# isarandi/metro-pose3d

Hardware: AMD Instinct MI355X
Metric: crops/sec (256x256, RN50 stride16) (higher is better)
Workload: dtype f16

## Files before the change

metro_pose3d_amd/csrc/conv_b1.hip:

```cpp
#include "metro_common.h"
#include "gfx950_prims.h"

namespace metro {

namespace b1 {
constexpr int NPROD = 8, NCONS = 4, NT = 64 * (NPROD + NCONS), TN = 64, K = 64, CB = 256, C2 = 64, NBUF = 3;
constexpr int X_BYTES = TN * 128;
constexpr int OUT_ROW = CB * 2 + 16;
constexpr int OUT_BYTES = TN * OUT_ROW;
constexpr int W1S_ROW = CB * 2 + 16;
static_assert(48 * W1S_ROW <= OUT_BYTES, "W1's stage must fit the second output tile");
template <bool REB>
struct Lay {
    static constexpr int NIN = REB ? 3 : 2;
    static constexpr int X_OFF = 0;
    static constexpr int OUT_OFF = NBUF * NIN * X_BYTES;
    static constexpr int PAR_OFF = OUT_OFF + 2 * OUT_BYTES;
    static constexpr int B3 = 0, BSC = 1024, BB = 2048, B2 = 3072, PRO = 3328, SC2 = 3584, SH2 = 4096, PAR_BYTES = 4608;
    static constexpr int W1T_OFF = PAR_OFF + PAR_BYTES;
    static constexpr int LDS = W1T_OFF + 8 * 64 * 16;
};
}

struct B1Args {
// ... 4 lines not shown
    const half_t* w_sc;
    const float* bias_sc;
    const half_t* pro_scale;
    const half_t* pro_shift;
    const half_t* in_b;
    const half_t* w_b;
    const float* bias_b;
    const half_t* w2;
    const float* bias2;
    const half_t* scale2;
    const half_t* shift2;
    half_t* out;
    half_t* out_sub;
    half_t* out2;
    int m_total, n_tiles;
    int h_out, w_out, lw_out, sub_off, h_sub, w_sub;
};

template <bool REB, int OUTM>
__global__ __launch_bounds__(b1::NT) void conv_b1_chain_kernel(B1Args a) {
    using namespace b1;
    using L = Lay<REB>;
    constexpr int NIN = L::NIN;
    extern __shared__ __attribute__((aligned(16))) char smem[];
    const unsigned smem_base = lds_offset_of(smem);
    const int tid = threadIdx.x;
    const int lane = tid & 63;
    const int wave = __builtin_amdgcn_readfirstlane(tid >> 6);
    const bool producer = wave < NPROD;
    const int G = gridDim.x;
    const int t0 = blockIdx.x;
    if (t0 >= a.n_tiles) return;
    const int T = (a.n_tiles - t0 + G - 1) / G;
    char* par = smem + L::PAR_OFF;
    {
        float* f = reinterpret_cast<float*>(par);
        if (tid < 256) {
            f[L::B3 / 4 + tid] = a.bias[tid];
            f[L::BSC / 4 + tid] = a.bias_sc[tid];
            if (REB) f[L::BB / 4 + tid] = a.bias_b[tid];
            reinterpret_cast<half_t*>(par + L::SC2)[tid] = a.scale2[tid];
            reinterpret_cast<half_t*>(par + L::SH2)[tid] = a.shift2[tid];
        }
        if (tid < 512) {
            const int ks = tid >> 6, ln = tid & 63;
            *reinterpret_cast<uint4*>(smem + L::W1T_OFF + tid * 16) =
                *reinterpret_cast<const uint4*>(a.w2 + (size_t)(48 + (ln & 15)) * CB + ks * 32 + (ln >> 4) * 8);
        }
        for (int c = tid; c < 48 * 32; c += NT)
            *reinterpret_cast<uint4*>(smem + L::OUT_OFF + OUT_BYTES + (c >> 5) * W1S_ROW + (c & 31) * 16) =
                *reinterpret_cast<const uint4*>(a.w2 + (size_t)(c >> 5) * CB + (c & 31) * 8);
        if (tid < 64) {
            f[L::B2 / 4 + tid] = a.bias2[tid];
            reinterpret_cast<half_t*>(par + L::PRO)[tid] = a.pro_scale[tid];
            reinterpret_cast<half_t*>(par + L::PRO)[64 + tid] = a.pro_shift[tid];
        }
    }
    const int frag_row = lane & 31, frag_half = lane >> 5;

    if (producer) {
        half8_t wf[4], wsf[4], wbf[4];
        static_assert(NPROD * W_STAGE_BYTES <= L::OUT_OFF + OUT_BYTES, "the staging scratch must stay below the second output tile (W1's stage)");
        load_w_frags_staged<K>(a.w + (size_t)wave * 32 * K, wf, smem + wave * W_STAGE_BYTES, lane);
        load_w_frags_staged<K>(a.w_sc + (size_t)wave * 32 * K, wsf, smem + wave * W_STAGE_BYTES, lane);
        if constexpr (REB) load_w_frags_staged<K>(a.w_b + (size_t)wave * 32 * K, wbf, smem + wave * W_STAGE_BYTES, lane);
#pragma unroll
        for (int kk = 0; kk < 4; ++kk) {
            asm volatile("" : "+v"(wf[kk]), "+v"(wsf[kk]));
            if constexpr (REB) asm volatile("" : "+v"(wbf[kk]));
        }
        const int xrow = wave * 8 + (lane >> 3);
        const int xoff = xrow * K + (((lane & 7) ^ swz<64>(xrow)) * 8);
        auto issue_tile = [&](int tile, int slot) {
            const size_t m0 = (size_t)tile * TN;
            const unsigned dst = smem_base + L::X_OFF + slot * NIN * X_BYTES + wave * 1024;
            dma16(a.in + m0 * K + xoff, __builtin_amdgcn_readfirstlane(dst));
            dma16(a.x_sc + m0 * K + xoff, __builtin_amdgcn_readfirstlane(dst + X_BYTES));
            if constexpr (REB) dma16(a.in_b + m0 * K + xoff, __builtin_amdgcn_readfirstlane(dst + 2 * X_BYTES));
        };
        wait_vm_and_barrier<0>();
        half8_t pre_s, pre_b;
        {
            const int ch = ((lane & 7) ^ swz<64>(xrow)) * 8;
            pre_s = *reinterpret_cast<const half8_t*>(par + L::PRO + ch * 2);
            pre_b = *reinterpret_cast<const half8_t*>(par + L::PRO + 128 + ch * 2);
        }
        issue_tile(t0, 0);
        if (T > 1) issue_tile(t0 + G, 1);
        floatx4 b3_r[4];
#pragma unroll
        for (int q = 0; q < 4; ++q) b3_r[q] = *reinterpret_cast<const floatx4*>(par + L::B3 + (wave * 32 + 8 * q + 4 * frag_half) * 4);
        const float* bias_sc_l = reinterpret_cast<const float*>(par + L::BSC);
        const float* bias_b_l = reinterpret_cast<const float*>(par + L::BB);
        const int boff0 = frag_row * 128 + ((frag_half ^ swz<64>(frag_row)) << 4);
        int slot = 0;
        for (int j = 0; j <= T; ++j) {
            if (j < T) {
                if (j + 1 < T) wait_vm<NIN>();
                else wait_vm<0>();
            }
            if (j < T) {
                half8_t* mine = reinterpret_cast<half8_t*>(smem + L::X_OFF + (slot * NIN + 1) * X_BYTES + wave * 1024 + lane * 16);
                const half8_t z = {};
                *mine = __builtin_elementwise_max(*mine * pre_s + pre_b, z);
            }
            wait_lgkm_and_barrier();
            if (j + 2 < T) issue_tile(t0 + (j + 2) * G, slot >= 1 ? slot - 1 : 2);
            if (j < T) {
                const char* xs = smem + L::X_OFF + slot * NIN * X_BYTES;
                char* ot = smem + L::OUT_OFF + (j & 1) * OUT_BYTES;
                floatx16 acc[2];
                half4_t xsum[2][4];
#pragma unroll
                for (int p = 0; p < 2; ++p)
#pragma unroll
                    for (int e = 0; e < 16; ++e) acc[p][e] = 0.f;
#pragma unroll
                for (int kk = 0; kk < 4; ++kk)
#pragma unroll
                    for (int p = 0; p < 2; ++p) {
                        const half8_t bs = *reinterpret_cast<const half8_t*>(xs + X_BYTES + p * 4096 + (boff0 ^ (kk << 5)));
// ... 158 lines not shown
```

metro_pose3d_amd/csrc/conv_pw64.hip:

```cpp
#include <cstdlib>
#include <type_traits>

#include "metro_common.h"
#include "gfx950_prims.h"

namespace metro {

struct Pw64Args {
    const half_t* in;
    const half_t* w;
    const float* bias;
    const half_t* pro_scale;
    const half_t* pro_shift;
    const half_t* residual;
    half_t* out;
    const half_t* w2;
    const float* bias2;
    const half_t* scale2;
    const half_t* shift2;
    half_t* out2;
    const half_t* x_sc;
    const half_t* w_sc;
    const float* bias_sc;
    const half_t* in_b;
// ... 7 lines not shown
};

namespace pw {
constexpr int NW = 8, NT = 512;
template <int K, int WM, int CB = 256>
struct Lay {
    static constexpr int WN = NW / WM;
    static constexpr int NI = CB / 32 / WM;
    static constexpr int TN = 32 * WN;
    static constexpr int KS = K / 64;
    static constexpr int SL_BYTES = TN * 128;
    static constexpr int X_BYTES = KS * SL_BYTES;
    static constexpr int XI = X_BYTES / 1024 / NW;
    static constexpr int CPR = CB / 8;
    static constexpr int RI = TN * CPR / NT;
    static constexpr int OUT_ROW = CB * 2 + 16;
    static constexpr int OUT_BYTES = TN * OUT_ROW;
    static constexpr int RES_BYTES = TN * CB * 2;
    static constexpr int C2 = CB == 512 ? 128 : 64;
    static constexpr int BIAS2_OFF = CB * 4, PRO_OFF = BIAS2_OFF + 512, BSC_OFF = PRO_OFF + 4 * K, BB_OFF = BSC_OFF + 1024;
    static constexpr int PAR_BYTES = BB_OFF + 1024;
    static constexpr int X_OFF = 0;
    static constexpr int OUT_OFF = X_OFF + 2 * X_BYTES;
    static constexpr int PAR_OFF = OUT_OFF + OUT_BYTES;
    static constexpr int RES_OFF = PAR_OFF + PAR_BYTES;
    static_assert(X_BYTES % (1024 * NW) == 0, "input tile must split evenly over the waves");
    static_assert(NI >= 1 && RI >= 1 && (TN * CPR) % NT == 0, "tile / thread mismatch");
};
template <int K, int WM, bool RES, int MODE2, bool PSC = false, int CB = 256, bool REB = false>
constexpr int lds_bytes() {
    return Lay<K, WM, CB>::RES_OFF + (RES ? 2 * Lay<K, WM, CB>::RES_BYTES : PSC ? (REB ? 4 : 2) * Lay<K, WM, CB>::X_BYTES
                                      : (MODE2 == 1 && K > 64) ? Lay<K, WM, CB>::C2 * (2 * K + 16) + Lay<K, WM, CB>::TN * (2 * Lay<K, WM, CB>::C2 + 16) : 0);
}
}

template <int BASE, int MAXX>
__device__ __forceinline__ void pw_wait_vm_plus(int extra) {
    if constexpr (MAXX == 0) {
        wait_vm<BASE>();
    } else {
        if (extra >= MAXX) wait_vm<BASE + MAXX>();
        else pw_wait_vm_plus<BASE, MAXX - 1>(extra);
    }
}
__device__ __forceinline__ void pw_wait_lgkm2(half8_t& r, half8_t& r2, int n) {
    switch (n) {
        case 0: asm volatile("s_waitcnt lgkmcnt(0)" : "+v"(r), "+v"(r2)); break;
        case 2: asm volatile("s_waitcnt lgkmcnt(2)" : "+v"(r), "+v"(r2)); break;
        case 4: asm volatile("s_waitcnt lgkmcnt(4)" : "+v"(r), "+v"(r2)); break;
        default: asm volatile("s_waitcnt lgkmcnt(6)" : "+v"(r), "+v"(r2)); break;
    }
}

template <int K, int WM, bool PRO, bool RES, int MODE2, bool RSUB = false, bool PSC = false, int CB = 256, bool REB = false, int OUTM = 0>
__global__ __launch_bounds__(pw::NT) void conv_pw64_kernel(Pw64Args a) {
    using namespace pw;
    using L = Lay<K, WM, CB>;
    static_assert((WM == 4 && K <= 128) || (WM == 8 && K <= 512), "weights must fit the register file as MFMA fragments");
    static_assert(CB == 256 || (CB == 512 && K == 128 && WM == 8 && RES && !PRO && !RSUB) ||
                      (CB == 512 && K == 256 && WM == 8 && !RES && PRO && MODE2 == 1),
                  "512-channel blocks: conv3 of block2, or block2's projection shortcut + conv1 pair");
    static_assert(MODE2 == 0 || (K == 64 && WM == 4) || (MODE2 == 2 && CB == 512) || (MODE2 == 1 && CB == 512 && K == 256),
                  "second outputs: block1 shapes, conv3 + next conv1 of block2, or block2's pair");
    static_assert(!PSC || (MODE2 == 2 && !PRO && !RES), "in-launch projection shortcut: conv3 + next conv1 of block1/unit_1");
    static_assert(!REB || PSC, "rebuilt residual: on top of the in-launch projection shortcut");
    static_assert(OUTM == 0 || (MODE2 == 2 && PSC), "outputs kept on chip: the conv3 + next conv1 launches of block1");
    constexpr int KK = K / 16, WN = L::WN, NI = L::NI, TN = L::TN, XI = L::XI, RI = L::RI;
    constexpr int X_BYTES = L::X_BYTES, X_OFF = L::X_OFF, OUT_OFF = L::OUT_OFF, PAR_OFF = L::PAR_OFF, RES_OFF = L::RES_OFF,
                  RES_BYTES = L::RES_BYTES, SL_BYTES = L::SL_BYTES, OUT_ROW = L::OUT_ROW, CPR = L::CPR, C2 = L::C2;
    extern __shared__ __attribute__((aligned(16))) char smem[];
    const unsigned smem_base = lds_offset_of(smem);
    constexpr int XS_OFF = RES_OFF;
    constexpr int XB_OFF = XS_OFF + 2 * X_BYTES;

    const int tid = threadIdx.x;
    const int lane = tid & 63;
    const int wave = __builtin_amdgcn_readfirstlane(tid >> 6);
    const int wm = wave / WN, wn = wave % WN;
    const int frag_row = lane & 31, frag_half = lane >> 5;
    const int halves = a.c_out / CB;
    const int G = gridDim.x / halves;
    int half, t;
    if ((gridDim.x & 7) == 0 && ((gridDim.x >> 3) % halves) == 0) {
        const int xcd = blockIdx.x & 7, j = blockIdx.x >> 3;
        half = j % halves;
        t = xcd * ((gridDim.x >> 3) / halves) + j / halves;
    } else {
        half = blockIdx.x % halves;
        t = blockIdx.x / halves;
    }
    if (t >= a.n_tiles) return;
    a.w += (size_t)half * CB * K;
    a.bias += half * CB;
    a.out += half * CB;
    if (RES) a.residual += half * CB;
    const int ldo = a.c_out;
    const half_t* zero = reinterpret_cast<const half_t*>(g_zero_page);

    half8_t wf[NI][KK];
    constexpr bool W_STAGED = K >= 128 && pw::lds_bytes<K, WM, RES, MODE2, PSC, CB, REB>() >= NW * W_STAGE_BYTES;
    constexpr int RG = C2 / 16;
    constexpr int NTW = TN / 16 / (NW / RG);
    constexpr int KS2 = CB / 32;
    half8_t w2r[MODE2 == 2 ? KS2 : 1];
    if constexpr (W_STAGED) {
#pragma unroll
        for (int i = 0; i < NI; ++i)
            load_w_frags_staged<K>(a.w + (size_t)((wm * NI + i) * 32) * K, wf[i], smem + wave * W_STAGE_BYTES, lane);
        if constexpr (MODE2 == 2) load_w_frags16_staged<CB>(a.w2 + (size_t)((wave % RG) * 16) * CB, w2r, smem + wave * W_STAGE_BYTES, lane);
        __syncthreads();
    } else {
#pragma unroll
        for (int i = 0; i < NI; ++i)
#pragma unroll
            for (int kk = 0; kk < KK; ++kk)
                wf[i][kk] = *reinterpret_cast<const half8_t*>(a.w + (size_t)((wm * NI + i) * 32 + frag_row) * K + kk * 16 + frag_half * 8);
    }
    half8_t wsf[NI][KK];
    if constexpr (PSC) {
#pragma unroll
        for (int i = 0; i < NI; ++i)
#pragma unroll
            for (int kk = 0; kk < KK; ++kk)
                wsf[i][kk] = *reinterpret_cast<const half8_t*>(a.w_sc + (size_t)((wm * NI + i) * 32 + frag_row) * K + kk * 16 + frag_half * 8);
    }
    half8_t wbf[NI][KK];
    if constexpr (REB) {
#pragma unroll
        for (int i = 0; i < NI; ++i)
#pragma unroll
            for (int kk = 0; kk < KK; ++kk)
                wbf[i][kk] = *reinterpret_cast<const half8_t*>(a.w_b + (size_t)((wm * NI + i) * 32 + frag_row) * K + kk * 16 + frag_half * 8);
    }
    constexpr bool W2_LDS = MODE2 == 1 && K > 64;
    constexpr bool PREPASS = PRO && W2_LDS;
    constexpr int W2_ROW = 2 * K + 16;
    constexpr int W2_OFF = RES_OFF;
    constexpr int O2_ROW = 2 * C2 + 16, O2_OFF = W2_OFF + C2 * W2_ROW;
    half8_t w2f[MODE2 == 1 && !W2_LDS ? KK : 1];
    if constexpr (MODE2 == 1 && !W2_LDS) {
        if (wave < 4) {
#pragma unroll
            for (int kk = 0; kk < KK; ++kk)
                w2f[kk] = *reinterpret_cast<const half8_t*>(a.w2 + (size_t)(wm * 32 + frag_row) * K + kk * 16 + frag_half * 8);
        }
    }
    if constexpr (W2_LDS) {
        for (int c = tid; c < C2 * (K / 8); c += NT) {
            const int r = c / (K / 8), q = c % (K / 8);
            *reinterpret_cast<uint4*>(smem + W2_OFF + r * W2_ROW + q * 16) = *reinterpret_cast<const uint4*>(a.w2 + (size_t)r * K + q * 8);
        }
    }
    const char* w2l = smem + W2_OFF + (wm * 32 + frag_row) * W2_ROW + frag_half * 16;
    float* bias_l = reinterpret_cast<float*>(smem + PAR_OFF);
    float* bias2_l = reinterpret_cast<float*>(smem + PAR_OFF + L::BIAS2_OFF);
    half_t* pro_l = reinterpret_cast<half_t*>(smem + PAR_OFF + L::PRO_OFF);
    if (tid < CB) bias_l[tid] = a.bias[tid];
    if (MODE2 != 0 && tid < C2) bias2_l[tid] = a.bias2[tid];
    if ((PRO || PSC) && tid < K) { pro_l[tid] = a.pro_scale[tid]; pro_l[K + tid] = a.pro_shift[tid]; }
    float* bias_sc_l = reinterpret_cast<float*>(smem + PAR_OFF + L::BSC_OFF);
    if (PSC && tid < 256) bias_sc_l[tid] = a.bias_sc[tid];
    float* bias_b_l = reinterpret_cast<float*>(smem + PAR_OFF + L::BB_OFF);
    if (REB && tid < 256) bias_b_l[tid] = a.bias_b[tid];
    const int ch = tid & (CPR - 1);
    half8_t sc2 = {}, sh2 = {};
    if constexpr (MODE2 == 2) {
        sc2 = *reinterpret_cast<const half8_t*>(a.scale2 + ch * 8);
        sh2 = *reinterpret_cast<const half8_t*>(a.shift2 + ch * 8);
        if constexpr (!W_STAGED) {
#pragma unroll
            for (int ks = 0; ks < KS2; ++ks)
                w2r[ks] = *reinterpret_cast<const half8_t*>(a.w2 + (size_t)((wave % RG) * 16 + (lane & 15)) * CB + ks * 32 + (lane >> 4) * 8);
        }
    }

    int xrow[XI], xoff[XI];
#pragma unroll
    for (int i = 0; i < XI; ++i) {
        const int q = i * NW + wave;
        xrow[i] = (q % (TN / 8)) * 8 + (lane >> 3);
        xoff[i] = xrow[i] * K + (q / (TN / 8)) * 64 + (((lane & 7) ^ swz<64>(xrow[i])) * 8);
    }
    auto issue_tile = [&](int tile, int buf) {
        const int m0 = tile * TN;
#pragma unroll
        for (int i = 0; i < XI; ++i) {
            const half_t* xs = (m0 + xrow[i] < a.m_total) ? a.in + (size_t)m0 * K + xoff[i] : zero;
            dma16(xs, __builtin_amdgcn_readfirstlane(smem_base + X_OFF + buf * X_BYTES + (i * NW + wave) * 1024));
            if constexpr (PSC) {
                const half_t* ss = (m0 + xrow[i] < a.m_total) ? a.x_sc + (size_t)m0 * K + xoff[i] : zero;
                dma16(ss, __builtin_amdgcn_readfirstlane(smem_base + XS_OFF + buf * X_BYTES + (i * NW + wave) * 1024));
            }
            if constexpr (REB) {
                const half_t* sb = (m0 + xrow[i] < a.m_total) ? a.in_b + (size_t)m0 * K + xoff[i] : zero;
                dma16(sb, __builtin_amdgcn_readfirstlane(smem_base + XB_OFF + buf * X_BYTES + (i * NW + wave) * 1024));
            }
        }
        if constexpr (RES) {
#pragma unroll
            for (int it = 0; it < RI; ++it) {
                const int c = it * NT + tid;
                const int m = m0 + c / CPR;
                size_t rrow = m;
                if constexpr (RSUB) {
                    const int hw = a.h_out * a.w_out;
                    const int img = m / hw, rem = m - img * hw;
                    const int ho = rem / a.w_out, wo = rem - ho * a.w_out;
                    rrow = ((size_t)img * a.res_h + a.res_off + a.res_stride * ho) * a.res_w + a.res_off + a.res_stride * wo;
                }
                const half_t* rs = m < a.m_total ? a.residual + rrow * ldo + (c & (CPR - 1)) * 8 : zero;
                dma16(rs, __builtin_amdgcn_readfirstlane(smem_base + RES_OFF + buf * RES_BYTES + it * 8192 + wave * 1024));
            }
        }
    };

    issue_tile(t, 0);
    constexpr int S2 = MODE2 == 2 ? NTW : (MODE2 == 1 && K > 64) ? 1 : 4;
    constexpr int RS = OUTM == 0 ? RI : 0;
    const bool two = MODE2 == 2 || (MODE2 == 1 && (wave < 4 || K > 64));
    bool prev_full = false;
    int prev_sub = 0;
    for (int it = 0;; ++it, t += G) {
        const int buf = it & 1;
        const int m0 = t * TN;
        if (it == 0 || !prev_full) wait_vm<0>();
        else if constexpr (OUTM == 2) pw_wait_vm_plus<S2, RI>(prev_sub);
        else if (two) wait_vm<RS + S2>();
        else wait_vm<RS>();
        wait_lgkm_and_barrier();
        if (t + G < a.n_tiles) issue_tile(t + G, buf ^ 1);
        prev_full = m0 + TN <= a.m_total;

        if constexpr (PREPASS) {
            static_assert(X_BYTES / 16 == 2 * NT, "two 16-byte chunks of the input tile per thread");
            const int c8 = lane & 7, prow = (wave & 3) * 8 + (lane >> 3);
            const half8_t z = {};
#pragma unroll
            for (int h = 0; h < 2; ++h) {
                const int sl = (wave >> 2) + 2 * h;
                half8_t* xp = reinterpret_cast<half8_t*>(smem + X_OFF + buf * X_BYTES + sl * SL_BYTES + prow * 128 + ((c8 ^ swz<64>(prow)) << 4));
                const half8_t sc = *reinterpret_cast<const half8_t*>(pro_l + sl * 64 + c8 * 8);
                const half8_t sh = *reinterpret_cast<const half8_t*>(pro_l + K + sl * 64 + c8 * 8);
                *xp = __builtin_elementwise_max(*xp * sc + sh, z);
            }
            wait_lgkm_and_barrier();
        }
        floatx16 acc[NI], acc2, accs[NI];
#pragma unroll
        for (int e = 0; e < 16; ++e) {
// ... 266 lines not shown
                         d.res_offset + 2 * (d.w_out - 1) < d.res_w;
    if (d.has_residual && !res_plain && !(f.form == ConvForm::Plain && res_sub && d.c_in <= 128)) return false;
    switch (f.form) {
        case ConvForm::Pair: {
            static const int pair256 = tuning_knob("METRO_PW_PAIR256", 1);
            return ((d.c_in == 64 && d.c_out == 320) || (pair256 && !classic_forms_forced() && d.c_in == 256 && d.c_out == 640)) &&
                   d.has_prologue && !d.has_residual && f.pair.relu2 == 1 && 5 * f.pair.c_out2 == d.c_out && f.pair.split == 4 * f.pair.c_out2;
        }
        case ConvForm::Next: {
            static const int next128 = tuning_knob("METRO_PW_NEXT128", 1);
            return ((d.c_in == 64 && d.c_out == 256 && f.next.c2 == 64) ||
                    (next128 && d.c_in == 128 && d.c_out == 512 && res_plain && f.next.c2 == 128)) && !d.has_prologue && d.has_residual;
        }
        case ConvForm::NextProj:
        case ConvForm::NextRebuild:
            return d.c_in == 64 && d.c_out == 256 && !d.has_prologue && !d.has_residual && f.next.c2 == 64 &&
                   (f.form == ConvForm::NextProj || b1_map_ok(d));
        case ConvForm::Plain:
            break;
    }
    if (d.c_in == 64 && d.c_out == 256) return (d.has_prologue != 0) != (d.has_residual != 0);
    static const int maxk = tuning_knob("METRO_PW_MAXK", 512);
    return (d.c_in == 128 || d.c_in == 256 || d.c_in == 512) && d.c_in <= maxk && d.c_out == 4 * d.c_in &&
           !d.has_prologue && d.has_residual;
}

template <int K, int WM, bool PRO, bool RES, int MODE2, bool RSUB = false, bool PSC = false, int CB = 256, bool REB = false, int OUTM = 0>
static int launch_pw(Pw64Args a, hipStream_t stream) {
    if (note_kernel("conv_pw64<k%d,wm%d%s%s%s%s%s%s%s%s>", K, WM, CB == 512 ? ",cb512" : "", PRO ? ",pro" : "", RES ? ",res" : "",
                    MODE2 == 1 ? ",pair" : MODE2 == 2 ? ",next" : "", RSUB ? ",ressub" : "", PSC ? ",projsc" : "", REB ? ",rebuild" : "",
                    OUTM == 1 ? ",noout" : OUTM == 2 ? ",subout" : ""))
        return METRO_OK;
    auto kern = conv_pw64_kernel<K, WM, PRO, RES, MODE2, RSUB, PSC, CB, REB, OUTM>;
    constexpr int lds = pw::lds_bytes<K, WM, RES, MODE2, PSC, CB, REB>();
    a.n_tiles = (a.m_total + pw::Lay<K, WM, CB>::TN - 1) / pw::Lay<K, WM, CB>::TN;
    static PerDeviceInt cap;
    int grid_cap = 0;
    if (const int st = ensure_dyn_lds_and_grid_cap(reinterpret_cast<const void*>(kern), pw::NT, lds, cap, "conv_pw64",
                                                   tuning_knob("METRO_PW64_BPC", 0) , &grid_cap))
        return st;
    const int halves = a.c_out / CB;
    int grid = a.n_tiles * halves < grid_cap ? a.n_tiles * halves : grid_cap;
    grid -= grid % halves;
    hipLaunchKernelGGL(kern, dim3(grid), dim3(pw::NT), lds, stream, a);
    return launch_status("conv_pw64");
}

int launch_conv_pw64(const MetroConvDesc& d, const void* in, const void* w, const float* bias, const void* ps,
                     const void* pb, const void* res, void* out, hipStream_t stream, const ConvFused& f) {
    const ConvRebuild& rb = f.rb;
    if ((f.form == ConvForm::NextRebuild || (f.form == ConvForm::NextProj && rb.out_mode == 1)) && !rb.classic &&
        conv_b1_chain_preferred() && b1_map_ok(d))
        return launch_conv_b1_chain(d, in, w, bias, out, stream, f);
    Pw64Args a;
    a.in = static_cast<const half_t*>(in);
    a.w = static_cast<const half_t*>(w);
    a.bias = bias;
    a.pro_scale = static_cast<const half_t*>(ps);
    a.pro_shift = static_cast<const half_t*>(pb);
    a.residual = d.has_residual ? static_cast<const half_t*>(res) : nullptr;
    a.out = static_cast<half_t*>(out);
    a.w2 = nullptr; a.bias2 = nullptr; a.scale2 = nullptr; a.shift2 = nullptr; a.out2 = nullptr;
    a.x_sc = nullptr; a.w_sc = nullptr; a.bias_sc = nullptr;
    a.in_b = nullptr; a.w_b = nullptr; a.bias_b = nullptr; a.out_sub = nullptr; a.sub_off = 0; a.h_sub = 0; a.w_sub = 0; a.lw_out = 0;
    a.m_total = d.n * d.h_out * d.w_out;
    a.n_tiles = 0;
    a.c_out = f.form == ConvForm::Pair ? f.pair.split : d.c_out;
// ... 39 lines not shown
```

metro_pose3d_amd/csrc/conv_pws.hip:

```cpp
#include "metro_common.h"
#include "gfx950_prims.h"

namespace metro {

struct PwsArgs {
    const half_t* in;
    const half_t* w;
    const float* bias;
    const half_t* residual;
    half_t* out;
    int m_total, n_tiles, c_out;
};

namespace pws {
constexpr int NW = 8, NT = 512, TN = 32, CB = 256, NBUF = 3;
constexpr int T_ROW = 80;
constexpr int T_BYTES = TN * T_ROW;
constexpr int R_BYTES = TN * 64;
template <int K>
struct Lay {
    static constexpr int KS = K / 64;
    static constexpr int SL_BYTES = TN * 128;
    static constexpr int X_BYTES = KS * SL_BYTES;
    static constexpr int NX = X_BYTES / 1024 / NW;
    static constexpr int X_OFF = 0;
    static constexpr int T_OFF = NBUF * X_BYTES;
    static constexpr int BIAS_OFF = T_OFF + NW * (T_BYTES + R_BYTES);
    static constexpr int LDS = BIAS_OFF + CB * 4;
    static_assert(X_BYTES % (1024 * NW) == 0, "operand tile must split evenly over the waves");
};
}

template <int K>
__global__ __launch_bounds__(pws::NT) void conv_pws_kernel(PwsArgs a) {
    using namespace pws;
    using L = Lay<K>;
    constexpr int KK = K / 16, NX = L::NX, X_BYTES = L::X_BYTES, SL_BYTES = L::SL_BYTES;
    extern __shared__ __attribute__((aligned(16))) char smem[];
    const unsigned smem_base = lds_offset_of(smem);
    const int tid = threadIdx.x;
    const int lane = tid & 63;
    const int wave = __builtin_amdgcn_readfirstlane(tid >> 6);
    const int frag_row = lane & 31, frag_half = lane >> 5;

    const int halves = a.c_out / CB;
    const int G = gridDim.x / halves;
    int half, t0;
    if ((gridDim.x & 7) == 0 && ((gridDim.x >> 3) % halves) == 0) {
        const int xcd = blockIdx.x & 7, j = blockIdx.x >> 3;
        half = j % halves;
        t0 = xcd * ((gridDim.x >> 3) / halves) + j / halves;
    } else {
        half = blockIdx.x % halves;
        t0 = blockIdx.x / halves;
    }
    if (t0 >= a.n_tiles) return;
    const int T = (a.n_tiles - t0 + G - 1) / G;
    const int ldo = a.c_out;
    const int co0 = half * CB + wave * 32;

    half8_t wf[KK];
    static_assert(L::BIAS_OFF >= NW * W_STAGE_BYTES, "the staging scratch must not reach the bias block");
    load_w_frags_staged<K>(a.w + (size_t)co0 * K, wf, smem + wave * W_STAGE_BYTES, lane);
#pragma unroll
    for (int kk = 0; kk < KK; ++kk) asm volatile("" : "+v"(wf[kk]));
    float* bias_l = reinterpret_cast<float*>(smem + L::BIAS_OFF);
    if (tid < CB) bias_l[tid] = a.bias[half * CB + tid];

    int xoff[NX];
#pragma unroll
    for (int i = 0; i < NX; ++i) {
        const int q = i * NW + wave;
        const int row = (q & 3) * 8 + (lane >> 3);
        xoff[i] = row * K + (q >> 2) * 64 + (((lane & 7) ^ swz<64>(row)) * 8);
    }
    auto issue_x = [&](int tile, int slot) {
        const half_t* src = a.in + (size_t)tile * TN * K;
#pragma unroll
        for (int i = 0; i < NX; ++i)
            dma16(src + xoff[i], __builtin_amdgcn_readfirstlane(smem_base + L::X_OFF + slot * X_BYTES + (i * NW + wave) * 1024));
    };
    char* tw = smem + L::T_OFF + wave * (T_BYTES + R_BYTES);
    const unsigned rw_lds = smem_base + L::T_OFF + wave * (T_BYTES + R_BYTES) + T_BYTES;
    const int rpx = lane >> 2, rch = lane & 3;
    auto issue_res = [&](int tile) {
        const half_t* src = a.residual + ((size_t)tile * TN + rpx) * ldo + co0 + rch * 8;
        dma16(src, __builtin_amdgcn_readfirstlane(rw_lds));
        dma16(src + (size_t)16 * ldo, __builtin_amdgcn_readfirstlane(rw_lds + 1024));
    };
    const int boff0 = frag_row * 128 + ((frag_half ^ swz<64>(frag_row)) << 4);

    wait_vm_and_barrier<0>();
    floatx4 bv[4];
#pragma unroll
    for (int q = 0; q < 4; ++q) bv[q] = *reinterpret_cast<const floatx4*>(bias_l + wave * 32 + 8 * q + 4 * frag_half);
    issue_x(t0, 0);
    if (T > 1) issue_x(t0 + G, 1);
    if (T > 1) wait_vm<NX>();
    else wait_vm<0>();
    if (wave >= 4) wait_lgkm_and_barrier();

    int slot = 0;
    for (int j = 0; j < T; ++j) {
        const int tile = t0 + j * G;
        wait_lgkm_and_barrier();
        issue_res(tile);
        if (j + 2 < T) issue_x(t0 + (j + 2) * G, slot >= 1 ? slot - 1 : 2);
        floatx16 acc;
#pragma unroll
        for (int e = 0; e < 16; ++e) acc[e] = 0.f;
        constexpr int DEPTH = 8;
        unsigned fbase[4];
#pragma unroll
        for (int c = 0; c < 4; ++c) fbase[c] = smem_base + L::X_OFF + slot * X_BYTES + (boff0 ^ (c << 5));
        half8_t fr[DEPTH];
#pragma unroll
        for (int kk = 0; kk < DEPTH; ++kk)
            asm volatile("ds_read_b128 %0, %1 offset:%2" : "=v"(fr[kk]) : "v"(fbase[kk & 3]), "n"((kk >> 2) * SL_BYTES));
#pragma unroll
        for (int kk = 0; kk < KK; ++kk) {
            if (KK - 1 - kk >= DEPTH - 1) asm volatile("s_waitcnt lgkmcnt(%1)" : "+v"(fr[kk % DEPTH]) : "n"(DEPTH - 1));
            else wait_lgkm_dyn(fr[kk % DEPTH], KK - 1 - kk);
            acc = __builtin_amdgcn_mfma_f32_32x32x16_f16(wf[kk], fr[kk % DEPTH], acc, 0, 0, 0);
            if (kk + DEPTH < KK)
                asm volatile("ds_read_b128 %0, %1 offset:%2" : "=v"(fr[kk % DEPTH]) : "v"(fbase[(kk + DEPTH) & 3]), "n"(((kk + DEPTH) >> 2) * SL_BYTES));
        }
        if (j + 2 < T) wait_vm<NX>();
        else wait_vm<0>();
        wait_lgkm_and_barrier();
#pragma unroll
        for (int q = 0; q < 4; ++q)
            *reinterpret_cast<half4_t*>(tw + frag_row * T_ROW + (8 * q + 4 * frag_half) * 2) = bias_cvt(acc, q, bv[q]);
// ... 58 lines not shown
```

metro_pose3d_amd/csrc/metro_common.h:

```cpp
#pragma once
#include <hip/hip_runtime.h>
#include <cstdarg>
#include <cstdint>
#include <cstdio>
#include <cstdlib>

#include "../../include/metro_hip.h"

namespace metro {

void set_error(const char* fmt, ...);
const char* get_error();

#define METRO_CHECK_ARG(cond, ...)                  \
    do {                                            \
        if (!(cond)) {                              \
            ::metro::set_error(__VA_ARGS__);        \
            return METRO_ERR_INVALID_ARG;           \
        }                                           \
    } while (0)

#define METRO_HIP_CHECK(expr)                                                              \
    do {                                                                                   \
        hipError_t _e = (expr);                                                            \
// ... 3 lines not shown
            return METRO_ERR_HIP;                                                          \
        }                                                                                  \
    } while (0)

inline int tuning_knob(const char* name, int dflt) {
#ifdef METRO_TUNING_KNOBS
    const char* e = getenv(name);
    return e ? atoi(e) : dflt;
#else
    (void)name;
    return dflt;
#endif
}

struct KernelNotes { int mode; char ids[1024]; };
KernelNotes& kernel_notes();
bool note_kernel(const char* fmt, ...) __attribute__((format(printf, 1, 2)));

typedef unsigned int metro_u32x4 __attribute__((ext_vector_type(4)));
template <int LEVEL = 1>
__device__ __forceinline__ void store_out16(void* p, uint4 v) {
#if defined(METRO_NT_STORES)
    if constexpr (METRO_NT_STORES >= LEVEL) {
        metro_u32x4 w = {v.x, v.y, v.z, v.w};
        __builtin_nontemporal_store(w, reinterpret_cast<metro_u32x4*>(p));
        return;
    }
#endif
    *reinterpret_cast<uint4*>(p) = v;
}

constexpr int W_STAGE_ROW = 272;
constexpr int W_STAGE_BYTES = 32 * W_STAGE_ROW;
template <int K, typename Frag>
__device__ __forceinline__ void load_w_frags_staged(const _Float16* __restrict__ rows , Frag* wf ,
                                                    char* scratch , int lane) {
    static_assert(K % 128 == 0 || K == 64, "whole 256-byte row pieces (K = 64: one 128-byte piece)");
    constexpr int PIECE = K >= 128 ? 128 : 64;
    constexpr int LPR = PIECE / 8;
    constexpr int RPI = 64 / LPR;
    const int lr = lane / LPR, lc = lane % LPR;
    const int fr = lane & 31, fh = lane >> 5;
#pragma unroll
    for (int c = 0; c < K / PIECE; ++c) {
#pragma unroll
        for (int j = 0; j < 32 / RPI; ++j)
            *reinterpret_cast<uint4*>(scratch + (j * RPI + lr) * W_STAGE_ROW + lc * 16) =
                *reinterpret_cast<const uint4*>(rows + (size_t)(j * RPI + lr) * K + c * PIECE + lc * 8);
        __builtin_amdgcn_wave_barrier();
#pragma unroll
        for (int k8 = 0; k8 < PIECE / 16; ++k8)
            wf[c * (PIECE / 16) + k8] = *reinterpret_cast<const Frag*>(scratch + fr * W_STAGE_ROW + k8 * 32 + fh * 16);
        __builtin_amdgcn_wave_barrier();
    }
}

template <int K, typename Frag>
__device__ __forceinline__ void load_w_frags16_staged(const _Float16* __restrict__ rows, Frag* wf , char* scratch, int lane) {
    static_assert(K % 128 == 0, "whole 256-byte row pieces");
    const int lr = lane >> 4, lc = lane & 15;
#pragma unroll
    for (int c = 0; c < K / 128; ++c) {
#pragma unroll
        for (int j = 0; j < 4; ++j)
            *reinterpret_cast<uint4*>(scratch + (j * 4 + lr) * W_STAGE_ROW + lc * 16) =
                *reinterpret_cast<const uint4*>(rows + (size_t)(j * 4 + lr) * K + c * 128 + lc * 8);
        __builtin_amdgcn_wave_barrier();
#pragma unroll
        for (int k4 = 0; k4 < 4; ++k4)
            wf[c * 4 + k4] = *reinterpret_cast<const Frag*>(scratch + (lane & 15) * W_STAGE_ROW + k4 * 64 + (lane >> 4) * 16);
        __builtin_amdgcn_wave_barrier();
    }
}

constexpr int METRO_MAX_DEVICES = 64;
struct PerDeviceInt { int v[METRO_MAX_DEVICES]; };

inline int current_device_slot(int* slot) {
    int dev = 0;
    const hipError_t e = hipGetDevice(&dev);
    if (e != hipSuccess || dev < 0 || dev >= METRO_MAX_DEVICES) {
        set_error("hipGetDevice: %s (device %d; at most %d devices per process)", hipGetErrorString(e), dev, METRO_MAX_DEVICES);
        return METRO_ERR_HIP;
    }
    *slot = dev;
    return METRO_OK;
}

inline int ensure_dyn_lds(const void* kern, int bytes, PerDeviceInt& done, const char* what) {
    int slot = 0;
    const int st = current_device_slot(&slot);
    if (st) return st;
    if (done.v[slot]) return METRO_OK;
    const hipError_t e = hipFuncSetAttribute(kern, hipFuncAttributeMaxDynamicSharedMemorySize, bytes);
    if (e != hipSuccess) {
        set_error("hipFuncSetAttribute(%s, %d B of LDS, device %d): %s", what, bytes, slot, hipGetErrorString(e));
        return METRO_ERR_HIP;
    }
    done.v[slot] = 1;
    return METRO_OK;
}

inline int ensure_dyn_lds_and_grid_cap(const void* kern, int threads, int bytes, PerDeviceInt& cap, const char* what,
                                       int max_blocks_per_cu, int* grid_cap) {
    int slot = 0;
// ... 228 lines not shown
```

Measured before the change: 48220.

## Overlap weight-fragment staging with input tile prefetch in pointwise conv kernels

```diff
diff --git a/metro_pose3d_amd/csrc/conv_b1.hip b/metro_pose3d_amd/csrc/conv_b1.hip
--- a/metro_pose3d_amd/csrc/conv_b1.hip
+++ b/metro_pose3d_amd/csrc/conv_b1.hip
@@ -60,6 +60,19 @@
     const int t0 = blockIdx.x;
     if (t0 >= a.n_tiles) return;
     const int T = (a.n_tiles - t0 + G - 1) / G;
+    const int xrow = (wave & (NPROD - 1)) * 8 + (lane >> 3);
+    const int xoff = xrow * K + (((lane & 7) ^ swz<64>(xrow)) * 8);
+    auto issue_tile = [&](int tile, int slot) {
+        const size_t m0 = (size_t)tile * TN;
+        const unsigned dst = smem_base + L::X_OFF + slot * NIN * X_BYTES + wave * 1024;
+        dma16(a.in + m0 * K + xoff, __builtin_amdgcn_readfirstlane(dst));
+        dma16(a.x_sc + m0 * K + xoff, __builtin_amdgcn_readfirstlane(dst + X_BYTES));
+        if constexpr (REB) dma16(a.in_b + m0 * K + xoff, __builtin_amdgcn_readfirstlane(dst + 2 * X_BYTES));
+    };
+    if (producer) {
+        issue_tile(t0, 0);
+        if (T > 1) issue_tile(t0 + G, 1);
+    }
     char* par = smem + L::PAR_OFF;
     {
         float* f = reinterpret_cast<float*>(par);
@@ -88,24 +101,23 @@
 
     if (producer) {
         half8_t wf[4], wsf[4], wbf[4];
-        static_assert(NPROD * W_STAGE_BYTES <= L::OUT_OFF + OUT_BYTES, "the staging scratch must stay below the second output tile (W1's stage)");
-        load_w_frags_staged<K>(a.w + (size_t)wave * 32 * K, wf, smem + wave * W_STAGE_BYTES, lane);
-        load_w_frags_staged<K>(a.w_sc + (size_t)wave * 32 * K, wsf, smem + wave * W_STAGE_BYTES, lane);
-        if constexpr (REB) load_w_frags_staged<K>(a.w_b + (size_t)wave * 32 * K, wbf, smem + wave * W_STAGE_BYTES, lane);
+        using WP = WPiece<K, 32>;
+        constexpr int STAGE_OFF = 2 * NIN * X_BYTES;
+        static_assert(STAGE_OFF + NPROD * WP::BYTES <= L::OUT_OFF + OUT_BYTES, "the staging scratch must stay below the second output tile (W1's stage)");
+        char* scratch = smem + STAGE_OFF + wave * WP::BYTES;
+        static_assert(WP::N == 1, "one piece per weight set");
+        WP pa, pb;
+        w_piece_fetch(pa, a.w + (size_t)wave * 32 * K, 0, lane);
+        w_piece_fetch(pb, a.w_sc + (size_t)wave * 32 * K, 0, lane);
+        w_frags_tail(pa, pb, wf, scratch, lane);
+        if constexpr (REB) w_piece_fetch(pa, a.w_b + (size_t)wave * 32 * K, 0, lane);
+        w_frags_tail(pb, pa, wsf, scratch, lane);
+        if constexpr (REB) w_frags_tail(pa, pb, wbf, scratch, lane);
 #pragma unroll
         for (int kk = 0; kk < 4; ++kk) {
             asm volatile("" : "+v"(wf[kk]), "+v"(wsf[kk]));
             if constexpr (REB) asm volatile("" : "+v"(wbf[kk]));
         }
-        const int xrow = wave * 8 + (lane >> 3);
-        const int xoff = xrow * K + (((lane & 7) ^ swz<64>(xrow)) * 8);
-        auto issue_tile = [&](int tile, int slot) {
-            const size_t m0 = (size_t)tile * TN;
-            const unsigned dst = smem_base + L::X_OFF + slot * NIN * X_BYTES + wave * 1024;
-            dma16(a.in + m0 * K + xoff, __builtin_amdgcn_readfirstlane(dst));
-            dma16(a.x_sc + m0 * K + xoff, __builtin_amdgcn_readfirstlane(dst + X_BYTES));
-            if constexpr (REB) dma16(a.in_b + m0 * K + xoff, __builtin_amdgcn_readfirstlane(dst + 2 * X_BYTES));
-        };
         wait_vm_and_barrier<0>();
         half8_t pre_s, pre_b;
         {
@@ -113,8 +125,6 @@
             pre_s = *reinterpret_cast<const half8_t*>(par + L::PRO + ch * 2);
             pre_b = *reinterpret_cast<const half8_t*>(par + L::PRO + 128 + ch * 2);
         }
-        issue_tile(t0, 0);
-        if (T > 1) issue_tile(t0 + G, 1);
         floatx4 b3_r[4];
 #pragma unroll
         for (int q = 0; q < 4; ++q) b3_r[q] = *reinterpret_cast<const floatx4*>(par + L::B3 + (wave * 32 + 8 * q + 4 * frag_half) * 4);
diff --git a/metro_pose3d_amd/csrc/conv_pw64.hip b/metro_pose3d_amd/csrc/conv_pw64.hip
--- a/metro_pose3d_amd/csrc/conv_pw64.hip
+++ b/metro_pose3d_amd/csrc/conv_pw64.hip
@@ -63,6 +63,17 @@
     return Lay<K, WM, CB>::RES_OFF + (RES ? 2 * Lay<K, WM, CB>::RES_BYTES : PSC ? (REB ? 4 : 2) * Lay<K, WM, CB>::X_BYTES
                                       : (MODE2 == 1 && K > 64) ? Lay<K, WM, CB>::C2 * (2 * K + 16) + Lay<K, WM, CB>::TN * (2 * Lay<K, WM, CB>::C2 + 16) : 0);
 }
+template <int K, int WM, bool RES, int MODE2, bool PSC = false, int CB = 256, bool REB = false>
+struct Stage {
+    using L = Lay<K, WM, CB>;
+    static constexpr int BASE = lds_bytes<K, WM, RES, MODE2, PSC, CB, REB>();
+    static constexpr bool ON = K >= 128 && BASE >= NW * W_STAGE_BYTES;
+    static constexpr int A_OFF = L::X_BYTES;
+    static constexpr int NA = (L::RES_OFF - A_OFF) / W_STAGE_BYTES < NW ? (L::RES_OFF - A_OFF) / W_STAGE_BYTES : NW;
+    static constexpr int B_OFF = L::RES_OFF + (RES ? L::RES_BYTES : 0);
+    static constexpr int TOTAL = ON && B_OFF + (NW - NA) * W_STAGE_BYTES > BASE ? B_OFF + (NW - NA) * W_STAGE_BYTES : BASE;
+    static_assert(TOTAL <= 160 * 1024, "LDS budget");
+};
 }
 
 template <int BASE, int MAXX>
@@ -128,83 +139,6 @@
     const int ldo = a.c_out;
     const half_t* zero = reinterpret_cast<const half_t*>(g_zero_page);
 
-    half8_t wf[NI][KK];
-    constexpr bool W_STAGED = K >= 128 && pw::lds_bytes<K, WM, RES, MODE2, PSC, CB, REB>() >= NW * W_STAGE_BYTES;
-    constexpr int RG = C2 / 16;
-    constexpr int NTW = TN / 16 / (NW / RG);
-    constexpr int KS2 = CB / 32;
-    half8_t w2r[MODE2 == 2 ? KS2 : 1];
-    if constexpr (W_STAGED) {
-#pragma unroll
-        for (int i = 0; i < NI; ++i)
-            load_w_frags_staged<K>(a.w + (size_t)((wm * NI + i) * 32) * K, wf[i], smem + wave * W_STAGE_BYTES, lane);
-        if constexpr (MODE2 == 2) load_w_frags16_staged<CB>(a.w2 + (size_t)((wave % RG) * 16) * CB, w2r, smem + wave * W_STAGE_BYTES, lane);
-        __syncthreads();
-    } else {
-#pragma unroll
-        for (int i = 0; i < NI; ++i)
-#pragma unroll
-            for (int kk = 0; kk < KK; ++kk)
-                wf[i][kk] = *reinterpret_cast<const half8_t*>(a.w + (size_t)((wm * NI + i) * 32 + frag_row) * K + kk * 16 + frag_half * 8);
-    }
-    half8_t wsf[NI][KK];
-    if constexpr (PSC) {
-#pragma unroll
-        for (int i = 0; i < NI; ++i)
-#pragma unroll
-            for (int kk = 0; kk < KK; ++kk)
-                wsf[i][kk] = *reinterpret_cast<const half8_t*>(a.w_sc + (size_t)((wm * NI + i) * 32 + frag_row) * K + kk * 16 + frag_half * 8);
-    }
-    half8_t wbf[NI][KK];
-    if constexpr (REB) {
-#pragma unroll
-        for (int i = 0; i < NI; ++i)
-#pragma unroll
-            for (int kk = 0; kk < KK; ++kk)
-                wbf[i][kk] = *reinterpret_cast<const half8_t*>(a.w_b + (size_t)((wm * NI + i) * 32 + frag_row) * K + kk * 16 + frag_half * 8);
-    }
-    constexpr bool W2_LDS = MODE2 == 1 && K > 64;
-    constexpr bool PREPASS = PRO && W2_LDS;
-    constexpr int W2_ROW = 2 * K + 16;
-    constexpr int W2_OFF = RES_OFF;
-    constexpr int O2_ROW = 2 * C2 + 16, O2_OFF = W2_OFF + C2 * W2_ROW;
-    half8_t w2f[MODE2 == 1 && !W2_LDS ? KK : 1];
-    if constexpr (MODE2 == 1 && !W2_LDS) {
-        if (wave < 4) {
-#pragma unroll
-            for (int kk = 0; kk < KK; ++kk)
-                w2f[kk] = *reinterpret_cast<const half8_t*>(a.w2 + (size_t)(wm * 32 + frag_row) * K + kk * 16 + frag_half * 8);
-        }
-    }
-    if constexpr (W2_LDS) {
-        for (int c = tid; c < C2 * (K / 8); c += NT) {
-            const int r = c / (K / 8), q = c % (K / 8);
-            *reinterpret_cast<uint4*>(smem + W2_OFF + r * W2_ROW + q * 16) = *reinterpret_cast<const uint4*>(a.w2 + (size_t)r * K + q * 8);
-        }
-    }
-    const char* w2l = smem + W2_OFF + (wm * 32 + frag_row) * W2_ROW + frag_half * 16;
-    float* bias_l = reinterpret_cast<float*>(smem + PAR_OFF);
-    float* bias2_l = reinterpret_cast<float*>(smem + PAR_OFF + L::BIAS2_OFF);
-    half_t* pro_l = reinterpret_cast<half_t*>(smem + PAR_OFF + L::PRO_OFF);
-    if (tid < CB) bias_l[tid] = a.bias[tid];
-    if (MODE2 != 0 && tid < C2) bias2_l[tid] = a.bias2[tid];
-    if ((PRO || PSC) && tid < K) { pro_l[tid] = a.pro_scale[tid]; pro_l[K + tid] = a.pro_shift[tid]; }
-    float* bias_sc_l = reinterpret_cast<float*>(smem + PAR_OFF + L::BSC_OFF);
-    if (PSC && tid < 256) bias_sc_l[tid] = a.bias_sc[tid];
-    float* bias_b_l = reinterpret_cast<float*>(smem + PAR_OFF + L::BB_OFF);
-    if (REB && tid < 256) bias_b_l[tid] = a.bias_b[tid];
-    const int ch = tid & (CPR - 1);
-    half8_t sc2 = {}, sh2 = {};
-    if constexpr (MODE2 == 2) {
-        sc2 = *reinterpret_cast<const half8_t*>(a.scale2 + ch * 8);
-        sh2 = *reinterpret_cast<const half8_t*>(a.shift2 + ch * 8);
-        if constexpr (!W_STAGED) {
-#pragma unroll
-            for (int ks = 0; ks < KS2; ++ks)
-                w2r[ks] = *reinterpret_cast<const half8_t*>(a.w2 + (size_t)((wave % RG) * 16 + (lane & 15)) * CB + ks * 32 + (lane >> 4) * 8);
-        }
-    }
-
     int xrow[XI], xoff[XI];
 #pragma unroll
     for (int i = 0; i < XI; ++i) {
@@ -246,6 +180,111 @@
     };
 
     issue_tile(t, 0);
+    float bias_v = 0.f, bias2_v = 0.f, bias_sc_v = 0.f, bias_b_v = 0.f;
+    half_t pro_s_v = 0, pro_b_v = 0;
+    if (tid < CB) bias_v = a.bias[tid];
+    if (MODE2 != 0 && tid < C2) bias2_v = a.bias2[tid];
+    if ((PRO || PSC) && tid < K) { pro_s_v = a.pro_scale[tid]; pro_b_v = a.pro_shift[tid]; }
+    if (PSC && tid < 256) bias_sc_v = a.bias_sc[tid];
+    if (REB && tid < 256) bias_b_v = a.bias_b[tid];
+
+    half8_t wf[NI][KK];
+    using ST = pw::Stage<K, WM, RES, MODE2, PSC, CB, REB>;
+    constexpr bool W_STAGED = ST::ON;
+    constexpr int RG = C2 / 16;
+    constexpr int NTW = TN / 16 / (NW / RG);
+    constexpr int KS2 = CB / 32;
+    half8_t w2r[MODE2 == 2 ? KS2 : 1];
+    if constexpr (W_STAGED) {
+        char* scratch = smem + (wave < ST::NA ? ST::A_OFF + wave * W_STAGE_BYTES : ST::B_OFF + (wave - ST::NA) * W_STAGE_BYTES);
+        static_assert(NI <= 2, "one or two weight sets per wave");
+        WPiece<K, 32> pa, pb;
+        WPiece<CB, 16> p2, q2;
+        const half_t* r0 = a.w + (size_t)(wm * NI * 32) * K;
+        const half_t* r1 = r0 + (size_t)32 * K;
+        const half_t* w2rows = a.w2 + (size_t)((wave % RG) * 16) * CB;
+        w_piece_fetch(pa, r0, 0, lane);
+        w_frags_head(pa, pb, r0, wf[0], scratch, lane);
+        if constexpr (NI == 2) w_piece_fetch(w_piece_free(pa, pb), r1, 0, lane);
+        else if constexpr (MODE2 == 2) w_piece_fetch(p2, w2rows, 0, lane);
+        w_frags_tail(pa, pb, wf[0], scratch, lane);
+        if constexpr (NI == 2) {
+            WPiece<K, 32>& sa = w_piece_free(pa, pb);
+            WPiece<K, 32>& sb = w_piece_last(pa, pb);
+            w_frags_head(sa, sb, r1, wf[NI - 1], scratch, lane);
+            if constexpr (MODE2 == 2) w_piece_fetch(p2, w2rows, 0, lane);
+            w_frags_tail(sa, sb, wf[NI - 1], scratch, lane);
+        }
+        if constexpr (MODE2 == 2) {
+            w_frags_head(p2, q2, w2rows, w2r, scratch, lane);
+            w_frags_tail(p2, q2, w2r, scratch, lane);
+        }
+        wait_lgkm_and_barrier();
+    } else {
+#pragma unroll
+        for (int i = 0; i < NI; ++i)
+#pragma unroll
+            for (int kk = 0; kk < KK; ++kk)
+                wf[i][kk] = *reinterpret_cast<const half8_t*>(a.w + (size_t)((wm * NI + i) * 32 + frag_row) * K + kk * 16 + frag_half * 8);
+    }
+    half8_t wsf[NI][KK];
+    if constexpr (PSC) {
+#pragma unroll
+        for (int i = 0; i < NI; ++i)
+#pragma unroll
+            for (int kk = 0; kk < KK; ++kk)
+                wsf[i][kk] = *reinterpret_cast<const half8_t*>(a.w_sc + (size_t)((wm * NI + i) * 32 + frag_row) * K + kk * 16 + frag_half * 8);
+    }
+    half8_t wbf[NI][KK];
+    if constexpr (REB) {
+#pragma unroll
+        for (int i = 0; i < NI; ++i)
+#pragma unroll
+            for (int kk = 0; kk < KK; ++kk)
+                wbf[i][kk] = *reinterpret_cast<const half8_t*>(a.w_b + (size_t)((wm * NI + i) * 32 + frag_row) * K + kk * 16 + frag_half * 8);
+    }
+    constexpr bool W2_LDS = MODE2 == 1 && K > 64;
+    constexpr bool PREPASS = PRO && W2_LDS;
+    constexpr int W2_ROW = 2 * K + 16;
+    constexpr int W2_OFF = RES_OFF;
+    constexpr int O2_ROW = 2 * C2 + 16, O2_OFF = W2_OFF + C2 * W2_ROW;
+    half8_t w2f[MODE2 == 1 && !W2_LDS ? KK : 1];
+    if constexpr (MODE2 == 1 && !W2_LDS) {
+        if (wave < 4) {
+#pragma unroll
+            for (int kk = 0; kk < KK; ++kk)
+                w2f[kk] = *reinterpret_cast<const half8_t*>(a.w2 + (size_t)(wm * 32 + frag_row) * K + kk * 16 + frag_half * 8);
+        }
+    }
+    if constexpr (W2_LDS) {
+        for (int c = tid; c < C2 * (K / 8); c += NT) {
+            const int r = c / (K / 8), q = c % (K / 8);
+            *reinterpret_cast<uint4*>(smem + W2_OFF + r * W2_ROW + q * 16) = *reinterpret_cast<const uint4*>(a.w2 + (size_t)r * K + q * 8);
+        }
+    }
+    const char* w2l = smem + W2_OFF + (wm * 32 + frag_row) * W2_ROW + frag_half * 16;
+    float* bias_l = reinterpret_cast<float*>(smem + PAR_OFF);
+    float* bias2_l = reinterpret_cast<float*>(smem + PAR_OFF + L::BIAS2_OFF);
+    half_t* pro_l = reinterpret_cast<half_t*>(smem + PAR_OFF + L::PRO_OFF);
+    if (tid < CB) bias_l[tid] = bias_v;
+    if (MODE2 != 0 && tid < C2) bias2_l[tid] = bias2_v;
+    if ((PRO || PSC) && tid < K) { pro_l[tid] = pro_s_v; pro_l[K + tid] = pro_b_v; }
+    float* bias_sc_l = reinterpret_cast<float*>(smem + PAR_OFF + L::BSC_OFF);
+    if (PSC && tid < 256) bias_sc_l[tid] = bias_sc_v;
+    float* bias_b_l = reinterpret_cast<float*>(smem + PAR_OFF + L::BB_OFF);
+    if (REB && tid < 256) bias_b_l[tid] = bias_b_v;
+    const int ch = tid & (CPR - 1);
+    half8_t sc2 = {}, sh2 = {};
+    if constexpr (MODE2 == 2) {
+        sc2 = *reinterpret_cast<const half8_t*>(a.scale2 + ch * 8);
+        sh2 = *reinterpret_cast<const half8_t*>(a.shift2 + ch * 8);
+        if constexpr (!W_STAGED) {
+#pragma unroll
+            for (int ks = 0; ks < KS2; ++ks)
+                w2r[ks] = *reinterpret_cast<const half8_t*>(a.w2 + (size_t)((wave % RG) * 16 + (lane & 15)) * CB + ks * 32 + (lane >> 4) * 8);
+        }
+    }
+
     constexpr int S2 = MODE2 == 2 ? NTW : (MODE2 == 1 && K > 64) ? 1 : 4;
     constexpr int RS = OUTM == 0 ? RI : 0;
     const bool two = MODE2 == 2 || (MODE2 == 1 && (wave < 4 || K > 64));
@@ -578,7 +617,7 @@
                     OUTM == 1 ? ",noout" : OUTM == 2 ? ",subout" : ""))
         return METRO_OK;
     auto kern = conv_pw64_kernel<K, WM, PRO, RES, MODE2, RSUB, PSC, CB, REB, OUTM>;
-    constexpr int lds = pw::lds_bytes<K, WM, RES, MODE2, PSC, CB, REB>();
+    constexpr int lds = pw::Stage<K, WM, RES, MODE2, PSC, CB, REB>::TOTAL;
     a.n_tiles = (a.m_total + pw::Lay<K, WM, CB>::TN - 1) / pw::Lay<K, WM, CB>::TN;
     static PerDeviceInt cap;
     int grid_cap = 0;
diff --git a/metro_pose3d_amd/csrc/conv_pws.hip b/metro_pose3d_amd/csrc/conv_pws.hip
--- a/metro_pose3d_amd/csrc/conv_pws.hip
+++ b/metro_pose3d_amd/csrc/conv_pws.hip
@@ -25,9 +25,12 @@
     static constexpr int NX = X_BYTES / 1024 / NW;
     static constexpr int X_OFF = 0;
     static constexpr int T_OFF = NBUF * X_BYTES;
-    static constexpr int BIAS_OFF = T_OFF + NW * (T_BYTES + R_BYTES);
+    static constexpr int STAGE_OFF = 2 * X_BYTES;
+    static constexpr int BIAS_OFF = T_OFF + NW * (T_BYTES + R_BYTES) > STAGE_OFF + NW * W_STAGE_BYTES ? T_OFF + NW * (T_BYTES + R_BYTES)
+                                                                                                      : STAGE_OFF + NW * W_STAGE_BYTES;
     static constexpr int LDS = BIAS_OFF + CB * 4;
     static_assert(X_BYTES % (1024 * NW) == 0, "operand tile must split evenly over the waves");
+    static_assert(LDS <= 160 * 1024, "LDS budget");
 };
 }
 
@@ -59,14 +62,6 @@
     const int ldo = a.c_out;
     const int co0 = half * CB + wave * 32;
 
-    half8_t wf[KK];
-    static_assert(L::BIAS_OFF >= NW * W_STAGE_BYTES, "the staging scratch must not reach the bias block");
-    load_w_frags_staged<K>(a.w + (size_t)co0 * K, wf, smem + wave * W_STAGE_BYTES, lane);
-#pragma unroll
-    for (int kk = 0; kk < KK; ++kk) asm volatile("" : "+v"(wf[kk]));
-    float* bias_l = reinterpret_cast<float*>(smem + L::BIAS_OFF);
-    if (tid < CB) bias_l[tid] = a.bias[half * CB + tid];
-
     int xoff[NX];
 #pragma unroll
     for (int i = 0; i < NX; ++i) {
@@ -80,6 +75,18 @@
         for (int i = 0; i < NX; ++i)
             dma16(src + xoff[i], __builtin_amdgcn_readfirstlane(smem_base + L::X_OFF + slot * X_BYTES + (i * NW + wave) * 1024));
     };
+    issue_x(t0, 0);
+    if (T > 1) issue_x(t0 + G, 1);
+
+    half8_t wf[KK];
+    static_assert(L::BIAS_OFF >= L::STAGE_OFF + NW * W_STAGE_BYTES, "the staging scratch must not reach the bias block");
+    const float bias_v = tid < CB ? a.bias[half * CB + tid] : 0.f;
+    load_w_frags_staged<K>(a.w + (size_t)co0 * K, wf, smem + L::STAGE_OFF + wave * W_STAGE_BYTES, lane);
+#pragma unroll
+    for (int kk = 0; kk < KK; ++kk) asm volatile("" : "+v"(wf[kk]));
+    float* bias_l = reinterpret_cast<float*>(smem + L::BIAS_OFF);
+    if (tid < CB) bias_l[tid] = bias_v;
+
     char* tw = smem + L::T_OFF + wave * (T_BYTES + R_BYTES);
     const unsigned rw_lds = smem_base + L::T_OFF + wave * (T_BYTES + R_BYTES) + T_BYTES;
     const int rpx = lane >> 2, rch = lane & 3;
@@ -94,10 +101,6 @@
     floatx4 bv[4];
 #pragma unroll
     for (int q = 0; q < 4; ++q) bv[q] = *reinterpret_cast<const floatx4*>(bias_l + wave * 32 + 8 * q + 4 * frag_half);
-    issue_x(t0, 0);
-    if (T > 1) issue_x(t0 + G, 1);
-    if (T > 1) wait_vm<NX>();
-    else wait_vm<0>();
     if (wave >= 4) wait_lgkm_and_barrier();
 
     int slot = 0;
diff --git a/metro_pose3d_amd/csrc/metro_common.h b/metro_pose3d_amd/csrc/metro_common.h
--- a/metro_pose3d_amd/csrc/metro_common.h
+++ b/metro_pose3d_amd/csrc/metro_common.h
@@ -59,45 +59,90 @@
 
 constexpr int W_STAGE_ROW = 272;
 constexpr int W_STAGE_BYTES = 32 * W_STAGE_ROW;
+template <int K, int ROWS>
+struct WPiece {
+    static_assert(K % 128 == 0 || K == 64, "whole 256-byte row pieces (K = 64: one 128-byte piece)");
+    static constexpr int PIECE = K >= 128 ? 128 : 64;
+    static constexpr int LPR = PIECE / 8;
+    static constexpr int RPI = 64 / LPR;
+    static constexpr int NLD = ROWS / RPI;
+    static constexpr int N = K / PIECE;
+    static constexpr int ROW = K == 64 ? 144 : W_STAGE_ROW;
+    static constexpr int BYTES = 32 * ROW;
+    metro_u32x4 v[NLD];
+};
+template <int K, int ROWS>
+__device__ __forceinline__ void w_piece_fetch(WPiece<K, ROWS>& p, const _Float16* __restrict__ rows , int c, int lane) {
+    using P = WPiece<K, ROWS>;
+    const int lr = lane / P::LPR, lc = lane % P::LPR;
+#pragma unroll
+    for (int j = 0; j < P::NLD; ++j)
+        p.v[j] = *reinterpret_cast<const metro_u32x4*>(rows + (size_t)(j * P::RPI + lr) * K + c * P::PIECE + lc * 8);
+}
+template <int K, typename Frag>
+__device__ __forceinline__ void w_piece_commit(const WPiece<K, 32>& p, Frag* wf , char* scratch, int lane) {
+    using P = WPiece<K, 32>;
+    const int lr = lane / P::LPR, lc = lane % P::LPR;
+    const int fr = lane & 31, fh = lane >> 5;
+#pragma unroll
+    for (int j = 0; j < P::NLD; ++j) *reinterpret_cast<metro_u32x4*>(scratch + (j * P::RPI + lr) * P::ROW + lc * 16) = p.v[j];
+    __builtin_amdgcn_wave_barrier();
+#pragma unroll
+    for (int k8 = 0; k8 < P::PIECE / 16; ++k8) wf[k8] = *reinterpret_cast<const Frag*>(scratch + fr * P::ROW + k8 * 32 + fh * 16);
+    __builtin_amdgcn_wave_barrier();
+}
+template <int K, typename Frag>
+__device__ __forceinline__ void w_piece_commit(const WPiece<K, 16>& p, Frag* wf, char* scratch, int lane) {
+    using P = WPiece<K, 16>;
+    static_assert(P::PIECE == 128, "whole 256-byte row pieces");
+    const int lr = lane >> 4, lc = lane & 15;
+#pragma unroll
+    for (int j = 0; j < P::NLD; ++j) *reinterpret_cast<metro_u32x4*>(scratch + (j * 4 + lr) * W_STAGE_ROW + lc * 16) = p.v[j];
+    __builtin_amdgcn_wave_barrier();
+#pragma unroll
+    for (int k4 = 0; k4 < 4; ++k4) wf[k4] = *reinterpret_cast<const Frag*>(scratch + (lane & 15) * W_STAGE_ROW + k4 * 64 + (lane >> 4) * 16);
+    __builtin_amdgcn_wave_barrier();
+}
+template <int K, int ROWS>
+__device__ __forceinline__ WPiece<K, ROWS>& w_piece_last(WPiece<K, ROWS>& p, WPiece<K, ROWS>& q) {
+    if constexpr (WPiece<K, ROWS>::N & 1) return p; else return q;
+}
+template <int K, int ROWS>
+__device__ __forceinline__ WPiece<K, ROWS>& w_piece_free(WPiece<K, ROWS>& p, WPiece<K, ROWS>& q) {
+    if constexpr (WPiece<K, ROWS>::N & 1) return q; else return p;
+}
+template <int K, int ROWS, int C = 0, typename Frag>
+__device__ __forceinline__ void w_frags_head(WPiece<K, ROWS>& cur , WPiece<K, ROWS>& nxt ,
+                                             const _Float16* __restrict__ rows, Frag* wf, char* scratch, int lane) {
+    using P = WPiece<K, ROWS>;
+    constexpr int FPP = ROWS == 32 ? P::PIECE / 16 : 4;
+    if constexpr (C + 1 < P::N) {
+        w_piece_fetch(nxt, rows, C + 1, lane);
+        w_piece_commit<K>(cur, wf + C * FPP, scratch, lane);
+        w_frags_head<K, ROWS, C + 1>(nxt, cur, rows, wf, scratch, lane);
+    }
+}
+template <int K, int ROWS, typename Frag>
+__device__ __forceinline__ void w_frags_tail(WPiece<K, ROWS>& p, WPiece<K, ROWS>& q, Frag* wf, char* scratch, int lane) {
+    using P = WPiece<K, ROWS>;
+    constexpr int FPP = ROWS == 32 ? P::PIECE / 16 : 4;
+    w_piece_commit<K>(w_piece_last(p, q), wf + (P::N - 1) * FPP, scratch, lane);
+}
 template <int K, typename Frag>
 __device__ __forceinline__ void load_w_frags_staged(const _Float16* __restrict__ rows , Frag* wf ,
                                                     char* scratch , int lane) {
-    static_assert(K % 128 == 0 || K == 64, "whole 256-byte row pieces (K = 64: one 128-byte piece)");
-    constexpr int PIECE = K >= 128 ? 128 : 64;
-    constexpr int LPR = PIECE / 8;
-    constexpr int RPI = 64 / LPR;
-    const int lr = lane / LPR, lc = lane % LPR;
-    const int fr = lane & 31, fh = lane >> 5;
-#pragma unroll
-    for (int c = 0; c < K / PIECE; ++c) {
-#pragma unroll
-        for (int j = 0; j < 32 / RPI; ++j)
-            *reinterpret_cast<uint4*>(scratch + (j * RPI + lr) * W_STAGE_ROW + lc * 16) =
-                *reinterpret_cast<const uint4*>(rows + (size_t)(j * RPI + lr) * K + c * PIECE + lc * 8);
-        __builtin_amdgcn_wave_barrier();
-#pragma unroll
-        for (int k8 = 0; k8 < PIECE / 16; ++k8)
-            wf[c * (PIECE / 16) + k8] = *reinterpret_cast<const Frag*>(scratch + fr * W_STAGE_ROW + k8 * 32 + fh * 16);
-        __builtin_amdgcn_wave_barrier();
-    }
+    WPiece<K, 32> p, q;
+    w_piece_fetch(p, rows, 0, lane);
+    w_frags_head(p, q, rows, wf, scratch, lane);
+    w_frags_tail(p, q, wf, scratch, lane);
 }
 
 template <int K, typename Frag>
 __device__ __forceinline__ void load_w_frags16_staged(const _Float16* __restrict__ rows, Frag* wf , char* scratch, int lane) {
-    static_assert(K % 128 == 0, "whole 256-byte row pieces");
-    const int lr = lane >> 4, lc = lane & 15;
-#pragma unroll
-    for (int c = 0; c < K / 128; ++c) {
-#pragma unroll
-        for (int j = 0; j < 4; ++j)
-            *reinterpret_cast<uint4*>(scratch + (j * 4 + lr) * W_STAGE_ROW + lc * 16) =
-                *reinterpret_cast<const uint4*>(rows + (size_t)(j * 4 + lr) * K + c * 128 + lc * 8);
-        __builtin_amdgcn_wave_barrier();
-#pragma unroll
-        for (int k4 = 0; k4 < 4; ++k4)
-            wf[c * 4 + k4] = *reinterpret_cast<const Frag*>(scratch + (lane & 15) * W_STAGE_ROW + k4 * 64 + (lane >> 4) * 16);
-        __builtin_amdgcn_wave_barrier();
-    }
+    WPiece<K, 16> p, q;
+    w_piece_fetch(p, rows, 0, lane);
+    w_frags_head(p, q, rows, wf, scratch, lane);
+    w_frags_tail(p, q, wf, scratch, lane);
 }
 
 constexpr int METRO_MAX_DEVICES = 64;
```

Measured after the change: 48310, median of 5. About the same (+0.2%).
